# zyj0021200/simpleImageCaptionZoo

Hardware: AMD Instinct MI355X
Metric: captions/sec (SCST step), BUTDDetection COCO14-size vocab (higher is better)
Workload: dtype f32

## Files before the change

include/icz.h:

```cpp
#ifndef ICZ_H_
#define ICZ_H_
#include <stddef.h>
#include <stdint.h>

#ifdef __cplusplus
extern "C" {
#endif

typedef enum {
    ICZ_OK = 0,
    ICZ_ERR_INVALID = -1,
    ICZ_ERR_HIP = -2,
    ICZ_ERR_STATE = -3,
    ICZ_ERR_NOMEM = -4
} icz_status;

const char* icz_last_error(void);
const char* icz_version(void);

typedef struct icz_butd icz_butd_t;

typedef struct {
    int32_t R;
    int32_t D;
// ... 233 lines not shown
int icz_rouge_lcs(const int32_t* hyp_tok, const int32_t* hyp_ptr, const int32_t* ref_tok, const int32_t* ref_ptr,
                  const int32_t* img_ref_ptr, int32_t n_img, int32_t* lcs_out, void* stream);

int icz_gemm_f32(int32_t layout, const float* X, int32_t ldx, const float* W, int32_t ldw, const float* bias,
                 float* C, int32_t ldc, int32_t M, int32_t N, int32_t K, int32_t nsplit, float* workspace,
                 size_t workspace_floats, void* stream);
size_t icz_gemm_workspace_floats(int32_t M, int32_t N);
int icz_gemm_set_big_cfg(int32_t cfg);
int icz_gemm_big_cfg_for(int32_t layout, int32_t M, int32_t N, int32_t K, int32_t nsplit);
int icz_gemm_tn_grouped(const float* dY, int32_t ldy, int32_t M, int32_t K, int32_t ngroups, const float* const* X, const int32_t* ldx,
                        const int32_t* cols, float* const* out, const int32_t* ldo, const int32_t* rows_live, void* stream);
int icz_gemm_tn_split_pick(int32_t M, int32_t N, int32_t K);
int icz_gemm_tn_split(const float* dY, int32_t ldy, int32_t M, const float* X, int32_t ldx, int32_t N, int32_t K, float* out, int32_t ldo,
                      float* workspace, size_t workspace_floats, const int32_t* rows_live, void* stream);
int icz_gemm_route_for(int32_t layout, int32_t M, int32_t N, int32_t nseg, const int32_t* K, int32_t nsplit);
int icz_gemm_tn_grouped_fits(int32_t M, int32_t K, int32_t ngroups, const int32_t* cols);
int icz_prof_begin(void);
int icz_prof_select(int32_t which);
int icz_prof_pair_overhead(void* stream, int32_t n, double* avg_us);
int icz_prof_end(double* avg_us, double* bytes_per_launch, double* flops_per_launch, long long* launches);
int icz_kprof_begin(void);
int icz_kprof_end(int32_t group, double* avg_us, long long* pairs);
int icz_prof_stream_rate(const void* buf, size_t bytes, int32_t reps, void* stream, double* gbs);

#ifdef __cplusplus
}
#endif
#endif
```

simpleimagecaptionzoo_amd/_lib.py:

```python
import ctypes as C
import os

_HERE = os.path.dirname(os.path.abspath(__file__))
LIB_PATH = os.path.join(_HERE, "libicz.so")


class IczError(RuntimeError):
    pass


GRAD_READY_CB = C.CFUNCTYPE(None, C.c_void_p, C.c_int32)


class ButdDims(C.Structure):
    _fields_ = [(n, C.c_int32) for n in ("R", "D", "H", "E", "A", "V", "max_rows", "max_len")]


BUTD_PARAM_FIELDS = (
    "embed_weight",
    "td_w_ih", "td_w_hh", "td_b_ih", "td_b_hh",
    "lm_w_ih", "lm_w_hh", "lm_b_ih", "lm_b_hh",
    "enc_att_v", "enc_att_g", "enc_att_b",
    "dec_att_v", "dec_att_g", "dec_att_b",
    "affine_v", "affine_g", "affine_b",
# ... 176 lines not shown
        "icz_prof_pair_overhead": (C.c_int, [vp, i32, C.POINTER(C.c_double)]),
        "icz_prof_end": (C.c_int, [C.POINTER(C.c_double), C.POINTER(C.c_double), C.POINTER(C.c_double), C.POINTER(C.c_longlong)]),
        "icz_kprof_begin": (C.c_int, []),
        "icz_kprof_end": (C.c_int, [i32, C.POINTER(C.c_double), C.POINTER(C.c_longlong)]),
        "icz_prof_stream_rate": (C.c_int, [vp, C.c_size_t, i32, vp, C.POINTER(C.c_double)]),
        "icz_adam_clamp_multi": (C.c_int, [i32, C.POINTER(vp), C.POINTER(vp), C.POINTER(vp), C.POINTER(vp), C.POINTER(i64), f32, f32, i32, vp]),
        "icz_gemm_f32": (C.c_int, [i32, vp, i32, vp, i32, vp, vp, i32, i32, i32, i32, i32, vp, C.c_size_t, vp]),
        "icz_gemm_workspace_floats": (C.c_size_t, [i32, i32]),
        "icz_gemm_set_big_cfg": (C.c_int, [i32]),
        "icz_gemm_big_cfg_for": (C.c_int, [i32, i32, i32, i32, i32]),
        "icz_gemm_tn_grouped": (C.c_int, [vp, i32, i32, i32, i32, vp, vp, vp, vp, vp, vp, vp]),
        "icz_gemm_tn_split_pick": (C.c_int, [i32, i32, i32]),
        "icz_gemm_tn_split": (C.c_int, [vp, i32, i32, vp, i32, i32, i32, vp, i32, vp, C.c_size_t, vp, vp]),
        "icz_gemm_route_for": (C.c_int, [i32, i32, i32, i32, vp, i32]),
        "icz_gemm_tn_grouped_fits": (C.c_int, [i32, i32, i32, vp]),
    }
    for name, (res, args) in sig.items():
        try:
            fn = getattr(L, name)
        except AttributeError as e:
            raise IczError("libicz.so lacks symbol %s (stale build?)" % name) from e
        fn.restype, fn.argtypes = res, args
    _lib = L
    return L


def check(status):
    if status != 0:
        raise IczError("libicz status %d: %s" % (status, lib().icz_last_error().decode()))

# ... 9 lines not shown
```

simpleimagecaptionzoo_amd/butd.py:

```python
import ctypes as C

import torch

from . import _lib
from ._lib import BUTD_PARAM_KEYS, ButdDims, ButdParams, Rng, check, lib, ptr, stream_ptr
from .handle import GraphDecoderHandle


def make_rng(seed=0, uniforms=None, emb_mask=None, att_mask=None, out_mask=None):
    r = Rng()
    r.seed = int(seed) & 0xFFFFFFFFFFFFFFFF
    keep = []
    for name, t, dt in (("uniforms", uniforms, torch.float32), ("emb_mask", emb_mask, torch.uint8),
                        ("att_mask", att_mask, torch.uint8), ("out_mask", out_mask, torch.uint8)):
        if t is not None:
            if t.dtype != dt or not t.is_cuda or not t.is_contiguous():
                raise _lib.IczError("%s must be a contiguous %s CUDA tensor" % (name, dt))
            setattr(r, name, t.data_ptr())
            keep.append(t)
    r._keep = keep
    return r


class ButdHandle(GraphDecoderHandle):
# ... 82 lines not shown
        N = W.shape[0]
    elif layout == "nn":
        M, K = X.shape
        N = W.shape[1]
    else:
        K, M = X.shape
        N = W.shape[1]
    out = torch.empty(M, N, device=X.device, dtype=torch.float32)
    ws = torch.empty(max(lib().icz_gemm_workspace_floats(M, N), max(nsplit, 1) * M * N), device=X.device,
                     dtype=torch.float32)
    check(lib().icz_gemm_f32(code, ptr(X), X.stride(0), ptr(W), W.stride(0), ptr(bias), ptr(out), N, M, N, K,
                             nsplit, ptr(ws), ws.numel(), stream_ptr()))
    return out


def gemm_set_big_cfg(cfg):
    check(lib().icz_gemm_set_big_cfg(int(cfg)))


def gemm_tn_grouped(dY, Xs, outs=None, rows_live=None):
    K, M = dY.shape
    n = len(Xs)
    if outs is None:
        outs = [torch.empty(M, x.shape[1], device=dY.device, dtype=torch.float32) for x in Xs]
    xp = (C.c_void_p * n)(*[x.data_ptr() for x in Xs])
    op = (C.c_void_p * n)(*[o.data_ptr() for o in outs])
    ldx = (C.c_int32 * n)(*[x.stride(0) for x in Xs])
    cols = (C.c_int32 * n)(*[x.shape[1] for x in Xs])
    ldo = (C.c_int32 * n)(*[o.stride(0) for o in outs])
    check(lib().icz_gemm_tn_grouped(ptr(dY), dY.stride(0), M, K, n, xp, ldx, cols, op, ldo, ptr(rows_live), stream_ptr()))
# ... 34 lines not shown
```

simpleimagecaptionzoo_amd/csrc/butd.hip:

```cpp
#include <vector>

#include "butd_impl.h"

namespace icz {

int Butd::init(const icz_butd_dims& d) {
    dims = d;
    ICZ_REQUIRE(d.R > 0 && d.R <= 64, "butd: R=%d must be in 1..64 (36 boxes / 49 grid cells)", d.R);
    ICZ_REQUIRE(d.D % 4 == 0 && d.H % 4 == 0 && d.E % 4 == 0 && d.A % 4 == 0, "butd: D,H,E,A must be multiples of 4");
    ICZ_REQUIRE(d.V > 3 && d.max_rows > 0 && d.max_len > 0, "butd: bad V/max_rows/max_len");
    const size_t rows = d.max_rows, H = d.H, D = d.D, E = d.E, A = d.A, V = d.V, R = d.R;
    ICZ_TRY(alloc((void**)&w_enc, sizeof(float) * A * D));
    ICZ_TRY(alloc((void**)&w_dec, sizeof(float) * A * H));
    ICZ_TRY(alloc((void**)&w_aff, sizeof(float) * A));
    const size_t Vp = pad_vocab(d.V);
    ICZ_TRY(alloc((void**)&w_pred, sizeof(float) * Vp * H));
    ICZ_TRY(alloc((void**)&n_enc, sizeof(float) * A));
    ICZ_TRY(alloc((void**)&n_dec, sizeof(float) * A));
    ICZ_TRY(alloc((void**)&n_aff, sizeof(float) * 4));
    ICZ_TRY(alloc((void**)&n_pred, sizeof(float) * V));
    ICZ_TRY(alloc((void**)&mean, sizeof(float) * rows * D));
    ICZ_TRY(alloc((void**)&premean, sizeof(float) * rows * 4 * H));
    ICZ_TRY(alloc((void**)&enc_ctx, sizeof(float) * rows * R * A));
    for (int i = 0; i < 2; ++i) {
// ... 13 lines not shown
    ICZ_TRY(alloc((void**)&it, sizeof(int64_t) * rows));
    ICZ_TRY(alloc_scalars(mem));
    size_t nmax = 4 * H;
    if (A > nmax) nmax = A;
    if (V > nmax) nmax = V;
    ws_floats = (size_t)TARGET_WGS * 4096 * 2 + rows * nmax;
    {
        const size_t kmax = 2 * H + (E > D ? E : D), r128 = rows < 128 ? rows : 128;
        const size_t need = (kmax / 256 + 1) * r128 * 4 * H;
        if (need > ws_floats) ws_floats = need;
    }
    ICZ_TRY(alloc((void**)&ws, sizeof(float) * ws_floats));
    ICZ_TRY(mem.synced());
    if (const char* e = getenv("ICZ_EARLY_OUT")) early_out = atoi(e) != 0;
    if (const char* e = getenv("ICZ_MERGE_SMALL")) { const int n = atoi(e); if (n >= 0 && n <= 32) merge_small = n; }
    return ICZ_OK;
}

int Butd::refresh(hipStream_t st) {
    ICZ_REQUIRE(bound, "butd: parameters not bound");
    const int A = dims.A, D = dims.D, H = dims.H, V = dims.V;
    WeightNormTable wt = {};
    int nb = 0;
    auto add = [&](const float* v, const float* g, float* w, float* norm, int rows, int cols) {
        wt.j[wt.count++] = {v, g, w, norm, rows, cols, nb};
        nb += cdiv(rows, 4);
    };
    add(P.enc_att_v, P.enc_att_g, w_enc, n_enc, A, D);
    add(P.dec_att_v, P.dec_att_g, w_dec, n_dec, A, H);
    add(P.affine_v, P.affine_g, w_aff, n_aff, 1, A);
    add(P.predict_v, P.predict_g, w_pred, n_pred, V, H);
    hipLaunchKernelGGL(weight_norm_multi_kernel, dim3(nb), dim3(256), 0, st, wt);
    ICZ_CHECK_HIP(hipGetLastError());
    fresh = true;
    wt_fresh = false;
    return ICZ_OK;
}

bool Butd::wt_possible() const {
    GemmArgs g = {};
    g.nseg = 1;
    g.seg[0] = {w_enc, w_enc, 4 * dims.H, 4 * dims.H, 4 * dims.H, nullptr};
    g.M = 64; g.N = dims.D + dims.H;
    GemmArgs p = g, q = g;
    p.N = q.N = dims.H;
    p.nseg = 2; p.seg[1] = p.seg[0];
    return dims.H % 64 == 0 && dims.D % 64 == 0 && gemm_resident_x3_fits(g) && gemm_resident_x3_pair_fits(p, q);
}

int Butd::refresh_transposes(hipStream_t st) {
    ICZ_REQUIRE(bound && wt_lm_ih, "butd: no transposed weight buffers");
    const int H = dims.H, D = dims.D, E = dims.E;
    TransposeTable tt = {};
    int nb = 0;
    auto add = [&](const float* src, int ld, int cols, float* dst) {
        tt.j[tt.count++] = {src, ld, 4 * H, cols, dst, nb};
        nb += (4 * H / 64) * (cols / 64);
    };
    add(P.lm_w_ih, D + H, D + H, wt_lm_ih);
    add(P.lm_w_hh, H, H, wt_lm_hh);
    add(P.td_w_ih, H + D + E, H, wt_td_ih_h2);
    add(P.td_w_hh, H, H, wt_td_hh);
// ... 231 lines not shown
        b->gc.clear();
    }
    b->P = *p;
    b->bound = true;
    b->fresh = false;
    return ICZ_OK;
}

int icz_butd_set_option(icz_butd_t* h, const char* name, int32_t value) {
    ICZ_REQUIRE(h && name, "icz_butd_set_option: null argument");
    Butd* b = reinterpret_cast<Butd*>(h);
    if (strcmp(name, "graphs") == 0) { b->use_graphs = value != 0; return ICZ_OK; }
    if (strcmp(name, "concurrent") == 0) { b->concurrent = value != 0; return ICZ_OK; }
    if (strcmp(name, "early_out") == 0) { b->early_out = value != 0; return ICZ_OK; }
    if (strcmp(name, "small_nt") == 0) { b->small_nt = value != 0; return ICZ_OK; }
    if (strcmp(name, "group_att") == 0) { b->group_att = value != 0; return ICZ_OK; }
    if (strcmp(name, "merge_small") == 0) {
        ICZ_REQUIRE(value >= 0 && value <= 32, "icz_butd_set_option: merge_small %d outside 0..32", value);
        b->merge_small = value;
        return ICZ_OK;
    }
    set_error("icz_butd_set_option: unknown option '%s'", name);
    return ICZ_ERR_INVALID;
}

int icz_butd_set_mask_sum_global(icz_butd_t* h, const float* mask_sum_global_dev, void* stream) {
    return set_norm_global("icz_butd_set_mask_sum_global", reinterpret_cast<Butd*>(h), mask_sum_global_dev, stream);
}

int icz_butd_set_grad_callback(icz_butd_t* h, icz_grad_ready_cb cb, void* user) {
// ... 40 lines not shown
```

simpleimagecaptionzoo_amd/csrc/butd_impl.h:

```cpp
#pragma once
#include <vector>
#include <stdint.h>

#include "decoder_core.h"

namespace icz {

struct StepIO {
    int rows;
    const float* feats;
    const int32_t* img_of_row;
    int rows_per_img;
    const int64_t* it;
    bool emb_ready;
    const float *h1_in, *c1_in, *h2_in, *c2_in;
    float *h1_out, *c1_out, *h2_out, *c2_out;
    float* emb_out;
    float* gates_td_out;
    float* gates_lm_out;
    float* dec_ctx_out;
    float* alpha_out;
    float* alpha_out2; int alpha2_stride;
    float* ctx_out;
    float* h2drop_out;
// ... 32 lines not shown
    icz_butd_params P;
    bool bound = false, fresh = false;
    DeviceBuffers mem;

    float *w_enc = nullptr, *w_dec = nullptr, *w_aff = nullptr, *w_pred = nullptr;
    float *n_enc = nullptr, *n_dec = nullptr, *n_aff = nullptr, *n_pred = nullptr;
    float *mean = nullptr, *premean = nullptr, *enc_ctx = nullptr;
    float *h1[2], *c1[2], *h2[2], *c2[2];
    float *emb = nullptr, *ctx = nullptr, *scores = nullptr, *alpha = nullptr, *h2drop = nullptr, *logits = nullptr;
    int64_t* it = nullptr;
    float* amax_val = nullptr; int* amax_idx = nullptr;
    float* ws = nullptr;
    size_t ws_floats = 0;
    float *wt_lm_ih = nullptr, *wt_lm_hh = nullptr, *wt_td_ih_h2 = nullptr, *wt_td_hh = nullptr;
    bool wt_fresh = false;
    bool wt_possible() const;
    int refresh_transposes(hipStream_t st);

    int alloc(void** p, size_t bytes) { return mem.alloc(p, bytes); }
    int init(const icz_butd_dims& d);
    int refresh(hipStream_t st);
    int gemm_nt(GemmArgs& g, int* nsplit_out, hipStream_t st);
    int prologue(const float* feats, int n_img, hipStream_t st);
    int step(const StepIO& s, hipStream_t st);
    int zero_state(int rows, int which, hipStream_t st);
    int greedy(const float* feats, int B, int max_len, int64_t* ids_out, float* alphas_out, hipStream_t st);

    GraphCache gc{24};
    bool use_graphs = false;
    bool concurrent = true;
    uintptr_t opt_bits() const {
        return (concurrent ? 1 : 0) + (early_out ? 2 : 0) + 4 * merge_small + (small_nt ? 256 : 0) + (group_att ? 512 : 0);
    }
    int greedy_impl(const float* feats, int B, int max_len, int64_t* ids_out, float* alphas_out, hipStream_t st);
    int sample_impl(const float* feats, int B, int T, int64_t* seq_out, float* logp_out, hipStream_t st);
    int greedy_chain(const float* feats, int B, int max_len, int64_t* ids_out, float* alphas_out, hipStream_t st, bool scst = false);
    int sample_chain(const float* feats, int B, int T, int64_t* seq_out, float* logp_out, hipStream_t st, int row0 = 0, int64_t* ids_out = nullptr);
    int rollouts(const float* feats, int B, int T, const icz_rng* r, int64_t* ids_out, int64_t* seq_out, float* logp_out, hipStream_t st);
    int rollouts_impl(const float* feats, int B, int T, int64_t* ids_out, int64_t* seq_out, float* logp_out, hipStream_t st);
    SideStream side;
    SideStream low;
    icz_grad_ready_cb grad_cb = nullptr; void* grad_cb_user = nullptr;
    int sample_backward_impl(const float* reward, const icz_butd_params& G, float* loss_out, float* mask_sum_out, hipStream_t st,
                             int phases = 0xF, bool fire_cb = true);
    bool bptt_joined = false;
    int merge_small = 8;
    int cur_rows = 0, cur_row0 = 0;
    bool early_out = true;
    bool bptt_early_out = false;
    bool small_nt = true;
    int cur_K = 1, cur_nimg = 0;
    bool group_att = false;

    const float* seam_feats = nullptr;
    int vocab() const override { return dims.V; }
    int row_capacity() const override { return dims.max_rows; }
    bool refreshed() const override { return fresh; }
    bool compact_step() const override { return true; }
    EmbSlot emb_slot() const override { return {P.embed_weight, emb, dims.E, 1}; }
    DeviceBuffers& buffers() override { return mem; }
    int prologue(const float* feats, int n_img, int k, const int32_t* img_of_row, hipStream_t st) override;
    int step(int rows, const int64_t* it, const int32_t* img_of_row, int rows_per_img, int cur, bool slabs, LogitsView* out,
             hipStream_t st) override;
    void gather(const int32_t* src_row, int rows, int fan, hipStream_t st) override;
// ... 27 lines not shown
```

simpleimagecaptionzoo_amd/csrc/butd_kernels.h:

```cpp
#pragma once
#include <stdlib.h>

#include "icz_common.h"
#include "rng.h"

namespace icz {
namespace {

__global__ __launch_bounds__(256) void weight_norm_kernel(const float* __restrict__ v, const float* __restrict__ g,
                                                          float* __restrict__ w, float* __restrict__ norm,
                                                          int rows, int cols) {
    const int lane = threadIdx.x & 63;
    const int row = blockIdx.x * 4 + (threadIdx.x >> 6);
    if (row >= rows) return;
    const float* vr = v + (size_t)row * cols;
    float ss = 0.f;
    for (int c = lane * 4; c < cols; c += 256) {
        f32x4 x = *reinterpret_cast<const f32x4*>(vr + c);
        ss += x[0] * x[0] + x[1] * x[1] + x[2] * x[2] + x[3] * x[3];
    }
    ss = wave_sum(ss);
    const float nrm = sqrtf(ss);
    const float s = g[row] / nrm;
    float* wr = w + (size_t)row * cols;
// ... 1194 lines not shown
    int lda_a;
    const float* dh_b; int ns_b; int lda_b;
    const float* dh_c; int ns_c; int lda_c;
    const float* dhdrop;
    const float* dc_in;
    const float* gates;
    const float* c_prev;
    const float* c_cur;
    float* dgates;
    float* dc_prev;
    int rows, H;
    int rows_a, rows_b, rows_c;
    int dc_in_rows;
    const int* live;
    const int* carry_live;
};
__global__ __launch_bounds__(256) void lstm_bwd_point_kernel(LstmBwdArgs a, DropCfg dc) {
    const int row = blockIdx.y;
    const int j = blockIdx.x * 256 + threadIdx.x;
    if (j >= a.H) return;
    const int H = a.H, G = 4 * H;
    const int lflag = live_flag(a.live), cflag = live_flag(a.carry_live);
    const float* g = a.gates + (size_t)row * G + j;
    const float gi = g[0], gf = g[H], gg = g[2 * H], go = g[3 * H];
    const float cc = a.c_cur[(size_t)row * H + j];
    const float cp = a.c_prev ? a.c_prev[(size_t)row * H + j] : 0.f;
    float dhd = 0.f;
    if (a.dhdrop) dhd = a.dhdrop[(size_t)row * H + j];
    if (flag_dead(lflag)) {
        float* o = a.dgates + (size_t)row * G + j;
        o[0] = 0.f; o[H] = 0.f; o[2 * H] = 0.f; o[3 * H] = 0.f;
        return;
    }
    const bool carry = cflag != 0;
    float dh = 0.f;
    if (a.dh_a && carry && row < a.rows_a) dh += sum_slabs1(a.dh_a, a.ns_a, (size_t)a.rows_a * a.lda_a, (size_t)row * a.lda_a + j);
    if (a.dh_b && row < a.rows_b) dh += sum_slabs1(a.dh_b, a.ns_b, (size_t)a.rows_b * a.lda_b, (size_t)row * a.lda_b + j);
    if (a.dh_c && row < a.rows_c) dh += sum_slabs1(a.dh_c, a.ns_c, (size_t)a.rows_c * a.lda_c, (size_t)row * a.lda_c + j);
    if (a.dhdrop) {
        float d = dhd;
        if (dc.mode) d = dc.keep((uint64_t)row * H + j) ? d * 2.0f : 0.f;
        dh += d;
    }
    const float dcin = (a.dc_in && carry && row < a.dc_in_rows) ? a.dc_in[(size_t)row * H + j] : 0.f;
    const float tc = tanhf(cc);
    const float dcv = dcin + dh * go * (1.f - tc * tc);
    float* o = a.dgates + (size_t)row * G + j;
    o[0] = dcv * gg * gi * (1.f - gi);
    o[H] = dcv * cp * gf * (1.f - gf);
    o[2 * H] = dcv * gi * (1.f - gg * gg);
    o[3 * H] = dh * tc * go * (1.f - go);
// ... 647 lines not shown
```

simpleimagecaptionzoo_amd/csrc/butd_train.hip:

```cpp
#include <math.h>

#include "butd_impl.h"

namespace icz {

static inline int round4(int x) { return pad_vocab(x); }

__global__ void sample_init_kernel(uint8_t* unf, int* nunf, int64_t* tok, int B, int T) {
    const int i = blockIdx.x * blockDim.x + threadIdx.x;
    if (i < B) { unf[i] = 1; tok[i] = 1; }
    if (i < T) nunf[i] = 0;
}

int Butd::ensure_train(int B, int T) {
    if (tb.B >= B && tb.T >= T) return ICZ_OK;
    ICZ_REQUIRE(B <= 2 * dims.max_rows, "butd: batch %d exceeds capacity %d", B, dims.max_rows);
    ICZ_REQUIRE(T <= XE_MAX_T, "butd: %d steps exceed the limit of %d", T, XE_MAX_T);
    if (tb.B > B) B = tb.B;
    if (tb.T > T) T = tb.T;
    if (dims.max_len > T) T = dims.max_len;
    if (!mem.training.empty()) {
        ICZ_TRY(mem.release_training(&gc));
        tb = TrainBuf();
        drop_loss_buffers();
    }
    if (!wt_lm_ih && wt_possible()) {
        const size_t G4 = 4 * (size_t)dims.H;
        ICZ_TRY(alloc((void**)&wt_lm_ih, sizeof(float) * G4 * (dims.D + dims.H)));
        ICZ_TRY(alloc((void**)&wt_lm_hh, sizeof(float) * G4 * dims.H));
        ICZ_TRY(alloc((void**)&wt_td_ih_h2, sizeof(float) * G4 * dims.H));
        ICZ_TRY(alloc((void**)&wt_td_hh, sizeof(float) * G4 * dims.H));
        wt_fresh = false;
    }
    DeviceBuffers::TrainingScope scope(mem);
    const size_t H = dims.H, D = dims.D, E = dims.E, A = dims.A, R = dims.R, V = dims.V;
    const size_t Vp = round4(dims.V);
    const size_t TB = (size_t)T * B;
    ICZ_TRY(alloc((void**)&tb.tok, sizeof(int64_t) * (TB + B)));
    ICZ_TRY(alloc((void**)&tb.emb, sizeof(float) * TB * E));
    ICZ_TRY(alloc((void**)&tb.h1, sizeof(float) * (TB + B) * H));
    ICZ_TRY(alloc((void**)&tb.c1, sizeof(float) * (TB + B) * H));
    ICZ_TRY(alloc((void**)&tb.h2, sizeof(float) * (TB + B) * H));
    ICZ_TRY(alloc((void**)&tb.c2, sizeof(float) * (TB + B) * H));
    ICZ_TRY(alloc((void**)&tb.gtd, sizeof(float) * TB * 4 * H));
    ICZ_TRY(alloc((void**)&tb.glm, sizeof(float) * TB * 4 * H));
    ICZ_TRY(alloc((void**)&tb.dec, sizeof(float) * TB * A));
// ... 440 lines not shown
        }
    }
    ICZ_TRY(side_branch());
    const bool ragged = rows_t[T - 1] < B || roff > 0;
    if (ragged) {
        ICZ_CHECK_HIP(hipMemsetAsync(tb.dGtd, 0, sizeof(float) * (size_t)TB * 4 * H, st));
        ICZ_CHECK_HIP(hipMemsetAsync(tb.dGlm, 0, sizeof(float) * (size_t)TB * 4 * H, st));
        ICZ_CHECK_HIP(hipMemsetAsync(tb.dDec, 0, sizeof(float) * (size_t)TB * A, st));
        ICZ_CHECK_HIP(hipMemsetAsync(tb.dS, 0, sizeof(float) * (size_t)TB * R, st));
    }

    auto loop = [&]() -> int {
    int cur = 0;
    int ns1 = 1, ns2 = 1, ns3 = 1, ns4 = 1;
    int bnext = 0;
    for (int t = T - 1; t >= 0; --t) {
        const int bt = rows_t[t];
        const size_t slot = (size_t)t * Bs + roff;
        const int* const live = (bptt_early_out && early_out && t > 0) ? nunf + (t - 1) : nullptr;
        const int* const carry_live = (bptt_early_out && early_out && t + 1 < T) ? nunf + t : nullptr;
        DropCfg d_out = make_drop(d_seed, cur_train, rng.out_mask, (size_t)B * H, RNG_OUT, t);
        DropCfg d_att = make_drop(d_seed, cur_train, rng.att_mask, (size_t)B * R * A, RNG_ATT, t);
        DropCfg d_off = {0, nullptr, nullptr, 0, 0};
        {
            LstmBwdArgs a = {};
            a.dh_a = bnext ? tb.X[2] : nullptr; a.ns_a = ns3; a.lda_a = H; a.rows_a = bnext;
            a.dhdrop = tb.dH2d + slot * H;
            a.dc_in = bnext ? tb.dc2[cur] : nullptr; a.dc_in_rows = bnext;
            a.gates = tb.glm + slot * 4 * H;
            a.c_prev = tb.c2 + slot * H; a.c_cur = tb.c2 + slot * H + sH;
            a.dgates = tb.dGlm + slot * 4 * H; a.dc_prev = tb.dc2[cur ^ 1];
            a.rows = bt; a.H = H; a.live = live; a.carry_live = carry_live;
            hipLaunchKernelGGL(lstm_bwd_point_kernel, dim3(cdiv(H, 256), bt), dim3(256), 0, st, a, d_out);
        }
        const bool rdg = wt_lm_ih && wt_fresh && bt > 32 && bt <= 64 && gemm_slab_floats(bt, D + H, 4 * H / 256) <= tb.xfloats &&
                         gemm_slab_floats(bt, H, 2 * (4 * H / 256)) <= tb.xfloats;
        const bool tdg = small_nt && wt_lm_ih && wt_fresh && bt <= 32;
        if (rdg) {
            GemmArgs g = {};
            g.nseg = 1;
            g.seg[0] = {tb.dGlm + slot * 4 * H, wt_lm_ih, 4 * H, 4 * H, 4 * H, nullptr};
            g.M = bt; g.N = D + H; g.out = tb.X[0]; g.ldo = D + H; g.live = live;
            g.nsplit = ns1 = gemm_resident_x3_nsplit(g);
            ICZ_REQUIRE(gemm_slab_floats(bt, D + H, ns1) <= tb.xfloats, "butd: slab buffer too small for the dgrad slabs");
            ICZ_TRY(gemm_f32(GEMM_NT, g, st));
        } else if (tdg) {
            GemmArgs g = {};
            g.nseg = 1;
            g.seg[0] = {tb.dGlm + slot * 4 * H, wt_lm_ih, 4 * H, 4 * H, 4 * H, nullptr};
            g.M = bt; g.N = D + H; g.out = tb.X[0]; g.ldo = D + H; g.live = live;
            ICZ_TRY(gemm_auto(GEMM_NT, g, tb.X[0], tb.xfloats, &ns1, st));
        } else {
            GemmArgs g = {};
            g.nseg = 1;
            g.seg[0] = {tb.dGlm + slot * 4 * H, P.lm_w_ih, 4 * H, D + H, 4 * H, nullptr};
            g.M = bt; g.N = D + H; g.out = tb.X[0]; g.ldo = D + H; g.live = live;
            ICZ_TRY(gemm_auto(GEMM_NN, g, tb.X[0], tb.xfloats, &ns1, st));
        }
        {
            const int dparts = cdiv(D, DALPHA_COLS);
            hipLaunchKernelGGL(att_bwd_dalpha_kernel, dim3(bt, dparts), dim3(256), 0, st, tb.X[0], ns1, D + H, bt, feats, R, D, tb.dalpha, live, imgk);
            AttBwdDdecArgs da = {enc_ctx, tb.dec + slot * A, w_aff, tb.alpha + slot * R, tb.dalpha, tb.dDec + slot * A, tb.dS + slot * R, R, A, dparts, live, imgk};
            hipLaunchKernelGGL(att_bwd_ddec_kernel, dim3(bt, cdiv(A, 256)), dim3(256), 0, st, da, d_att);
            GemmArgs g = {};
            g.nseg = 1;
            g.seg[0] = {tb.dDec + slot * A, w_dec, A, H, A, nullptr};
            g.M = bt; g.N = H; g.out = tb.X[1]; g.ldo = H; g.live = live;
            ICZ_TRY(gemm_auto(GEMM_NN, g, tb.X[1], tb.xfloats, &ns2, st));
        }
        {
            LstmBwdArgs a = {};
            a.dh_a = bnext ? tb.X[3] : nullptr; a.ns_a = ns4; a.lda_a = H; a.rows_a = bnext;
            a.dh_b = tb.X[0] + D; a.ns_b = ns1; a.lda_b = D + H; a.rows_b = bt;
            a.dh_c = tb.X[1]; a.ns_c = ns2; a.lda_c = H; a.rows_c = bt;
            a.dc_in = bnext ? tb.dc1[cur] : nullptr; a.dc_in_rows = bnext;
            a.gates = tb.gtd + slot * 4 * H;
            a.c_prev = tb.c1 + slot * H; a.c_cur = tb.c1 + slot * H + sH;
            a.dgates = tb.dGtd + slot * 4 * H; a.dc_prev = tb.dc1[cur ^ 1];
            a.rows = bt; a.H = H; a.live = live; a.carry_live = carry_live;
            hipLaunchKernelGGL(lstm_bwd_point_kernel, dim3(cdiv(H, 256), bt), dim3(256), 0, st, a, d_off);
        }
        if (t > 0 && rdg) {
            GemmArgs g3 = {}, g4 = {};
            g3.nseg = 2;
            g3.seg[0] = {tb.dGlm + slot * 4 * H, wt_lm_hh, 4 * H, 4 * H, 4 * H, nullptr};
            g3.seg[1] = {tb.dGtd + slot * 4 * H, wt_td_ih_h2, 4 * H, 4 * H, 4 * H, nullptr};
            g3.M = bt; g3.N = H; g3.out = tb.X[2]; g3.ldo = H; g3.live = live;
            g4.nseg = 1; g4.live = live;
            g4.seg[0] = {tb.dGtd + slot * 4 * H, wt_td_hh, 4 * H, 4 * H, 4 * H, nullptr};
            g4.M = bt; g4.N = H; g4.out = tb.X[3]; g4.ldo = H;
            ns3 = gemm_resident_x3_nsplit(g3); ns4 = gemm_resident_x3_nsplit(g4);
            ICZ_REQUIRE(gemm_slab_floats(bt, H, ns3) <= tb.xfloats, "butd: slab buffer too small for the dgrad slabs");
            ICZ_TRY(gemm_resident_x3_pair(g3, g4, st));
        } else if (t > 0 && tdg) {
            {
                GemmArgs g = {};
                g.nseg = 2;
// ... 14 lines not shown
                GemmArgs g = {};
                g.nseg = 2;
                g.seg[0] = {tb.dGlm + slot * 4 * H, P.lm_w_hh, 4 * H, H, 4 * H, nullptr};
                g.seg[1] = {tb.dGtd + slot * 4 * H, P.td_w_ih, 4 * H, H + D + E, 4 * H, nullptr};
                g.M = bt; g.N = H; g.out = tb.X[2]; g.ldo = H; g.live = live;
                ICZ_TRY(gemm_auto(GEMM_NN, g, tb.X[2], tb.xfloats, &ns3, st));
            }
            {
                GemmArgs g = {};
                g.nseg = 1;
                g.seg[0] = {tb.dGtd + slot * 4 * H, P.td_w_hh, 4 * H, H, 4 * H, nullptr};
                g.M = bt; g.N = H; g.out = tb.X[3]; g.ldo = H; g.live = live;
                ICZ_TRY(gemm_auto(GEMM_NN, g, tb.X[3], tb.xfloats, &ns4, st));
            }
        }
        bnext = bt;
        cur ^= 1;
    }
    return ICZ_OK;
    };
    const int s_loop = loop();
    if (grad_cb || s_loop != ICZ_OK) {
        ICZ_CHECK_HIP(hipStreamWaitEvent(st, ev_join, 0));
        bptt_joined = true;
    }
    if (s_loop != ICZ_OK) return s_loop;
    }
    if ((phases & 1) && grad_cb && fire_cb) grad_cb(grad_cb_user, 0);
    const int ldtd = H + D + E, ldlm = D + H;
    const bool tail_side = phases == 0xF && !grad_cb && concurrent;
// ... 218 lines not shown
```

simpleimagecaptionzoo_amd/csrc/gemm_f32.h:

```cpp
#pragma once
#include "icz_common.h"

namespace icz {

constexpr int GEMM_MAX_SEG = 4;
constexpr int GEMM_BM = 64, GEMM_BN = 64, GEMM_BK = 64;

enum GemmLayout { GEMM_NT = 0, GEMM_NN = 1, GEMM_TN = 2 };

struct GemmSeg {
    const float* A;
    const float* B;
    int lda, ldb;
    int K;
    const int64_t* gather;
};

struct GemmArgs {
    GemmSeg seg[GEMM_MAX_SEG];
    int nseg;
    int M, N;
    float* out;
    int ldo;
    const float* bias;
    int nsplit;
    int chunks_per_split;
    int accumulate;
    int spread;
    const int* live;
    const int* rows_live;
};

int gemm_f32(GemmLayout layout, const GemmArgs& a, hipStream_t stream);
int gemm_route(GemmLayout layout, const GemmArgs& a);
int gemm_pick_split(const GemmArgs& a, int target_wgs, GemmLayout layout = GEMM_NT);
int gemm_pick_split_balanced(const GemmArgs& a, GemmLayout layout, size_t slab_capacity_floats);
size_t gemm_slab_floats(int M, int N, int nsplit);
int gemm_normalize_split(GemmLayout layout, const GemmArgs& a, int nsplit);
int gemm_fit_split(GemmLayout layout, const GemmArgs& a, int nsplit, size_t capacity_floats);

bool gemm_resident_x3_fits(const GemmArgs& a);
int gemm_resident_x3_stages(const GemmArgs& a);
int gemm_resident_x3_nsplit(const GemmArgs& a);
int gemm_resident_x3(const GemmArgs& a, hipStream_t stream);
bool gemm_resident_x3_pair_fits(const GemmArgs& a, const GemmArgs& b);
int gemm_resident_x3_pair(const GemmArgs& a, const GemmArgs& b, hipStream_t stream);
int gemm_predict(const float* x, int H, const float* w_pred, const float* bias, int rows, int V, int Vp, float* logits, int ldl,
                 float* ws, size_t ws_cap_floats, int* pred_nsplit, hipStream_t st, const int* live = nullptr);

int gemm_big_x3(GemmLayout layout, const GemmArgs& a, int cfg, hipStream_t stream);
int gemm_big_cfg(GemmLayout layout, const GemmArgs& a);
int gemm_big_switch();
void gemm_set_big_cfg(int cfg);
constexpr int GEMM_MAX_COLGROUPS = 4;
struct GemmColGroup { const float* B; int ldb; int cols; float* out; int ldo; };
bool gemm_tn_grouped_fits(int M, int K, const GemmColGroup* groups, int ngroups);
int gemm_tn_grouped(const float* dY, int ldy, int M, int K, const GemmColGroup* groups, int ngroups, const int* rows_live, hipStream_t stream);

// ... 7 lines not shown
```

simpleimagecaptionzoo_amd/csrc/gemm_f32.hip:

```cpp
#include <stdlib.h>

#include <array>
#include <mutex>
#include <set>
#include <vector>

#include "gemm_f32.h"
#include "butd_kernels.h"

namespace icz {

static int total_chunks(const GemmArgs& a, int bk = GEMM_BK) {
    int t = 0;
    for (int s = 0; s < a.nseg; ++s) t += cdiv(a.seg[s].K, bk);
    return t;
}

template <int BK>
struct ChunkCursorT {
    int seg, k0;
    const float* A; const float* B;
    int lda, ldb, K;
    __device__ __forceinline__ void load_seg(const GemmArgs& a) {
        const GemmSeg& g = a.seg[seg];
// ... 1215 lines not shown
    if (g.nsplit > 1) {
        ICZ_REQUIRE(workspace, "icz_gemm_f32: split-K needs a workspace");
        ICZ_REQUIRE(gemm_slab_floats(M, N, g.nsplit) <= workspace_floats, "icz_gemm_f32: workspace of %zu floats too small for %d slabs of %dx%d", workspace_floats, g.nsplit, M, N);
        ICZ_REQUIRE(ldc == N, "icz_gemm_f32: split-K path needs ldc == N");
        g.out = workspace; g.bias = nullptr;
        ICZ_TRY(gemm_f32((GemmLayout)layout, g, st));
        size_t MN = (size_t)M * N;
        ICZ_REQUIRE(MN % 4 == 0, "icz_gemm_f32: M*N must be a multiple of 4 for the split-K reduce");
        hipLaunchKernelGGL(slab_reduce_kernel, dim3(cdiv((int)(MN / 4), 256)), dim3(256), 0, st, workspace, g.nsplit, MN, N, bias, C);
        ICZ_CHECK_HIP(hipGetLastError());
        return ICZ_OK;
    }
    return gemm_f32((GemmLayout)layout, g, st);
}

int icz_gemm_set_big_cfg(int32_t cfg) {
    ICZ_REQUIRE(cfg >= -2 && cfg <= 5, "icz_gemm_set_big_cfg: %d", cfg);
    gemm_set_big_cfg(cfg);
    return ICZ_OK;
}

int icz_gemm_big_cfg_for(int32_t layout, int32_t M, int32_t N, int32_t K, int32_t nsplit) {
    if (layout < 0 || layout > 2 || M <= 0 || N <= 0 || K <= 0) return -1;
    GemmArgs g = {};
    g.nseg = 1;
    g.seg[0].K = K;
    g.M = M; g.N = N; g.nsplit = nsplit > 0 ? nsplit : 1;
    return gemm_big_cfg((GemmLayout)layout, g);
}

// ... 51 lines not shown
```

simpleimagecaptionzoo_amd/csrc/gemm_resident_x3.hip:

```cpp
#include <stdlib.h>

#include <type_traits>

#include "gemm_f32.h"

namespace icz {

template <int I, int N, class F>
__device__ __forceinline__ void sk_static_for(F&& f) {
    if constexpr (I < N) {
        f(std::integral_constant<int, I>{});
        sk_static_for<I + 1, N>(f);
    }
}

typedef __attribute__((ext_vector_type(8))) __bf16 sk_bf16x8;
typedef __attribute__((ext_vector_type(4))) uint32_t sk_u32x4;
typedef __attribute__((ext_vector_type(2))) uint32_t sk_u32x2;

__device__ __forceinline__ uint32_t sk_cvt_pk_bf16(float lo, float hi) {
    uint32_t r;
    asm("v_cvt_pk_bf16_f32 %0, %1, %2" : "=v"(r) : "v"(lo), "v"(hi));
    return r;
}
// ... 491 lines not shown
}

template <int D, bool STAMPS = false>
__global__ __launch_bounds__(256) void gemm_resident_x3_m128_kernel(GemmArgs a) {
    resident_x3_m128_body<D, STAMPS>(a, blockIdx.x);
}
constexpr size_t rs_m128_lds_bytes() { return (size_t)3 * 128 * rs_pb(2) * 2; }

static int rs_total_stages(const GemmArgs& a) {
    int tot = 0;
    for (int s = 0; s < a.nseg; ++s) tot += a.seg[s].K / SK_BK;
    return tot;
}
int gemm_resident_x3_stages(const GemmArgs& a) {
    const int tot = rs_total_stages(a);
    if (gemm_switches().resident_k512 && a.M <= 64 && tot % 8 == 0) return 8;
    return tot % 4 == 0 ? 4 : 0;
}
static bool rs_shape_ok(const GemmArgs& a) {
    if (!gemm_switches().resident_x3 || a.M <= 32 || a.M > (gemm_switches().resident_m128 ? 128 : 64) || a.N % 4 || a.accumulate) return false;
    for (int s = 0; s < a.nseg; ++s)
        if (a.seg[s].K % SK_BK || a.seg[s].gather) return false;
    return rs_total_stages(a) >= 8 && gemm_resident_x3_stages(a) > 0;
}
bool gemm_resident_x3_fits(const GemmArgs& a) { return a.N >= 2048 && rs_shape_ok(a); }
int gemm_resident_x3_nsplit(const GemmArgs& a) { return rs_total_stages(a) / gemm_resident_x3_stages(a); }

template <int NSR, bool STAMPS>
static int rs_launch(const GemmArgs& a, hipStream_t stream) {
    constexpr size_t lds = rs_lds_bytes<4, NSR>();
    static bool attr = false;
    if (!attr) {
        ICZ_CHECK_HIP(hipFuncSetAttribute(reinterpret_cast<const void*>(gemm_resident_x3_kernel<4, NSR, 2, 3, STAMPS>), hipFuncAttributeMaxDynamicSharedMemorySize, (int)lds));
        attr = true;
    }
    hipLaunchKernelGGL((gemm_resident_x3_kernel<4, NSR, 2, 3, STAMPS>), dim3(cdiv(a.N, 256) * a.nsplit), dim3(256), lds, stream, a);
    ICZ_CHECK_HIP(hipGetLastError());
    return ICZ_OK;
}

#ifndef RS_K512_D
#define RS_K512_D 3
#endif
template <bool STAMPS>
static int rs_launch_k512(const GemmArgs& a, hipStream_t stream) {
    constexpr size_t lds = rs_lds_bytes<4, 4>();
    static bool attr = false;
    if (!attr) {
        ICZ_CHECK_HIP(hipFuncSetAttribute(reinterpret_cast<const void*>(gemm_resident_x3_kernel<4, 8, 1, RS_K512_D, STAMPS, 4>), hipFuncAttributeMaxDynamicSharedMemorySize, (int)lds));
        attr = true;
    }
// ... 18 lines not shown
#ifdef ICZ_DEV
static unsigned long long* g_sk_stamps = nullptr;
static int rs_dev_env(const char* name) { const char* e = getenv(name); return e ? atoi(e) : 0; }
#endif

int gemm_resident_x3(const GemmArgs& a_in, hipStream_t stream) {
    GemmArgs a = a_in;
    const int nsr = gemm_resident_x3_stages(a);
    ICZ_REQUIRE(rs_shape_ok(a) && a.nsplit == gemm_resident_x3_nsplit(a) && a.chunks_per_split == nsr,
                "gemm_resident_x3: launch does not match the kernel's fixed decomposition (nsplit %d)", a.nsplit);
    ICZ_REQUIRE(a.nsplit > 1 || a.ldo >= a.N, "gemm_resident_x3: output row stride %d below N = %d", a.ldo, a.N);
#ifdef ICZ_DEV
    if (rs_dev_env("ICZ_DEV_STAMPS")) {
        if (!g_sk_stamps) ICZ_CHECK_HIP(hipMalloc((void**)&g_sk_stamps, sizeof(unsigned long long) * 32 * 4096));
        a.bias = reinterpret_cast<const float*>(g_sk_stamps);
        return a.M > 64 ? rs_launch_m128<true>(a, stream) : (nsr == 8 ? rs_launch_k512<true>(a, stream) : rs_launch<4, true>(a, stream));
    }
#endif
    return a.M > 64 ? rs_launch_m128<false>(a, stream) : (nsr == 8 ? rs_launch_k512<false>(a, stream) : rs_launch<4, false>(a, stream));
}

bool gemm_resident_x3_pair_fits(const GemmArgs& a, const GemmArgs& b) {
    return a.M <= 64 && b.M <= 64 && rs_shape_ok(a) && rs_shape_ok(b) && gemm_resident_x3_stages(a) == gemm_resident_x3_stages(b) && a.N >= 512 && b.N >= 512;
}
int gemm_resident_x3_pair(const GemmArgs& a_in, const GemmArgs& b_in, hipStream_t stream) {
    ICZ_REQUIRE(gemm_resident_x3_pair_fits(a_in, b_in), "gemm_resident_x3_pair: shapes outside the kernel's decomposition");
    GemmPair g;
    g.a = a_in; g.b = b_in;
    const int nsr = gemm_resident_x3_stages(g.a), tilew = nsr == 8 ? 128 : 256;
    for (GemmArgs* p : {&g.a, &g.b}) {
        p->nsplit = gemm_resident_x3_nsplit(*p);
        p->chunks_per_split = nsr;
        p->bias = nullptr;
        ICZ_REQUIRE(p->out && p->nsplit > 1, "gemm_resident_x3_pair: slab output expected");
// ... 44 lines not shown
```

Baseline: 11850.

## Regroup BPTT dgrad GEMMs by concatenating LSTM weight transposes

Stores the transposed LSTM weights contiguously, so the LM input and recurrent dgrads become one wider GEMM (N = D+2H), and the TD input/recurrent dgrads one GEMM of width 2H. It adds a narrow resident-kernel form that uses one tile per workgroup, giving that 2H GEMM more workgroups. The pointwise backward kernel gains a second carried-gradient source so it can read the split slabs. The aim is fewer launches and better occupancy per timestep, at the cost of more slab memory and extra routing logic.

```diff
diff --git a/include/icz.h b/include/icz.h
--- a/include/icz.h
+++ b/include/icz.h
@@ -271,6 +271,8 @@
 int icz_gemm_tn_split(const float* dY, int32_t ldy, int32_t M, const float* X, int32_t ldx, int32_t N, int32_t K, float* out, int32_t ldo,
                       float* workspace, size_t workspace_floats, const int32_t* rows_live, void* stream);
 int icz_gemm_route_for(int32_t layout, int32_t M, int32_t N, int32_t nseg, const int32_t* K, int32_t nsplit);
+int icz_gemm_resident_slabs(const float* X, int32_t ldx, const float* W, int32_t ldw, int32_t M, int32_t N, int32_t K, int32_t form,
+                            float* slabs, size_t slab_floats, int32_t* nsplit_out, void* stream);
 int icz_gemm_tn_grouped_fits(int32_t M, int32_t K, int32_t ngroups, const int32_t* cols);
 int icz_prof_begin(void);
 int icz_prof_select(int32_t which);
diff --git a/simpleimagecaptionzoo_amd/_lib.py b/simpleimagecaptionzoo_amd/_lib.py
--- a/simpleimagecaptionzoo_amd/_lib.py
+++ b/simpleimagecaptionzoo_amd/_lib.py
@@ -214,6 +214,7 @@
         "icz_gemm_tn_split": (C.c_int, [vp, i32, i32, vp, i32, i32, i32, vp, i32, vp, C.c_size_t, vp, vp]),
         "icz_gemm_route_for": (C.c_int, [i32, i32, i32, i32, vp, i32]),
         "icz_gemm_tn_grouped_fits": (C.c_int, [i32, i32, i32, vp]),
+        "icz_gemm_resident_slabs": (C.c_int, [vp, i32, vp, i32, i32, i32, i32, i32, vp, C.c_size_t, C.POINTER(i32), vp]),
     }
     for name, (res, args) in sig.items():
         try:
diff --git a/simpleimagecaptionzoo_amd/butd.py b/simpleimagecaptionzoo_amd/butd.py
--- a/simpleimagecaptionzoo_amd/butd.py
+++ b/simpleimagecaptionzoo_amd/butd.py
@@ -120,6 +120,16 @@
     return out
 
 
+def gemm_resident_slabs(X, W, form=0, max_slabs=64):
+    M, K = X.shape
+    N = W.shape[0]
+    ws = torch.empty(max_slabs * M * N, device=X.device, dtype=torch.float32)
+    ns = C.c_int32(0)
+    check(lib().icz_gemm_resident_slabs(ptr(X), X.stride(0), ptr(W), W.stride(0), M, N, K, int(form), ptr(ws), ws.numel(), C.byref(ns),
+                                        stream_ptr()))
+    return ws[:ns.value * M * N].view(ns.value, M, N)
+
+
 def gemm_set_big_cfg(cfg):
     check(lib().icz_gemm_set_big_cfg(int(cfg)))
 
diff --git a/simpleimagecaptionzoo_amd/csrc/butd.hip b/simpleimagecaptionzoo_amd/csrc/butd.hip
--- a/simpleimagecaptionzoo_amd/csrc/butd.hip
+++ b/simpleimagecaptionzoo_amd/csrc/butd.hip
@@ -51,6 +51,7 @@
     ICZ_TRY(mem.synced());
     if (const char* e = getenv("ICZ_EARLY_OUT")) early_out = atoi(e) != 0;
     if (const char* e = getenv("ICZ_MERGE_SMALL")) { const int n = atoi(e); if (n >= 0 && n <= 32) merge_small = n; }
+    if (const char* e = getenv("ICZ_BPTT_REGROUP")) { const int n = atoi(e); if (n >= 0 && n <= 2) bptt_regroup = n; }
     return ICZ_OK;
 }
 
@@ -79,10 +80,20 @@
     g.nseg = 1;
     g.seg[0] = {w_enc, w_enc, 4 * dims.H, 4 * dims.H, 4 * dims.H, nullptr};
     g.M = 64; g.N = dims.D + dims.H;
-    GemmArgs p = g, q = g;
-    p.N = q.N = dims.H;
-    p.nseg = 2; p.seg[1] = p.seg[0];
-    return dims.H % 64 == 0 && dims.D % 64 == 0 && gemm_resident_x3_fits(g) && gemm_resident_x3_pair_fits(p, q);
+    GemmArgs g2 = g, n = g;
+    g2.N = dims.D + 2 * dims.H;
+    n.N = 2 * dims.H; n.form = GEMM_FORM_NARROW;
+    return dims.H % 64 == 0 && dims.D % 64 == 0 && gemm_resident_x3_fits(g) && gemm_resident_x3_fits(g2) && gemm_resident_x3_takes(n);
+}
+bool Butd::wt_pair_possible() const {
+    GemmArgs p = {};
+    p.nseg = 2;
+    p.seg[0] = {w_enc, w_enc, 4 * dims.H, 4 * dims.H, 4 * dims.H, nullptr};
+    p.seg[1] = p.seg[0];
+    p.M = 64; p.N = dims.H;
+    GemmArgs q = p;
+    q.nseg = 1;
+    return gemm_resident_x3_pair_fits(p, q);
 }
 
 int Butd::refresh_transposes(hipStream_t st) {
@@ -344,6 +355,11 @@
     if (strcmp(name, "concurrent") == 0) { b->concurrent = value != 0; return ICZ_OK; }
     if (strcmp(name, "early_out") == 0) { b->early_out = value != 0; return ICZ_OK; }
     if (strcmp(name, "small_nt") == 0) { b->small_nt = value != 0; return ICZ_OK; }
+    if (strcmp(name, "bptt_regroup") == 0) {
+        ICZ_REQUIRE(value >= 0 && value <= 2, "icz_butd_set_option: bptt_regroup %d outside 0..2", value);
+        b->bptt_regroup = value;
+        return ICZ_OK;
+    }
     if (strcmp(name, "group_att") == 0) { b->group_att = value != 0; return ICZ_OK; }
     if (strcmp(name, "merge_small") == 0) {
         ICZ_REQUIRE(value >= 0 && value <= 32, "icz_butd_set_option: merge_small %d outside 0..32", value);
diff --git a/simpleimagecaptionzoo_amd/csrc/butd_impl.h b/simpleimagecaptionzoo_amd/csrc/butd_impl.h
--- a/simpleimagecaptionzoo_amd/csrc/butd_impl.h
+++ b/simpleimagecaptionzoo_amd/csrc/butd_impl.h
@@ -70,7 +70,9 @@
     size_t ws_floats = 0;
     float *wt_lm_ih = nullptr, *wt_lm_hh = nullptr, *wt_td_ih_h2 = nullptr, *wt_td_hh = nullptr;
     bool wt_fresh = false;
+    bool wt_pair = false;
     bool wt_possible() const;
+    bool wt_pair_possible() const;
     int refresh_transposes(hipStream_t st);
 
     int alloc(void** p, size_t bytes) { return mem.alloc(p, bytes); }
@@ -86,7 +88,7 @@
     bool use_graphs = false;
     bool concurrent = true;
     uintptr_t opt_bits() const {
-        return (concurrent ? 1 : 0) + (early_out ? 2 : 0) + 4 * merge_small + (small_nt ? 256 : 0) + (group_att ? 512 : 0);
+        return (concurrent ? 1 : 0) + (early_out ? 2 : 0) + 4 * merge_small + (small_nt ? 256 : 0) + (group_att ? 512 : 0) + 1024 * bptt_regroup;
     }
     int greedy_impl(const float* feats, int B, int max_len, int64_t* ids_out, float* alphas_out, hipStream_t st);
     int sample_impl(const float* feats, int B, int T, int64_t* seq_out, float* logp_out, hipStream_t st);
@@ -104,6 +106,7 @@
     int cur_rows = 0, cur_row0 = 0;
     bool early_out = true;
     bool bptt_early_out = false;
+    int bptt_regroup = 1;
     bool small_nt = true;
     int cur_K = 1, cur_nimg = 0;
     bool group_att = false;
diff --git a/simpleimagecaptionzoo_amd/csrc/butd_kernels.h b/simpleimagecaptionzoo_amd/csrc/butd_kernels.h
--- a/simpleimagecaptionzoo_amd/csrc/butd_kernels.h
+++ b/simpleimagecaptionzoo_amd/csrc/butd_kernels.h
@@ -1232,6 +1232,8 @@
     int dc_in_rows;
     const int* live;
     const int* carry_live;
+    const float* dh_a2; int ns_a2;
+    int lda_a2;
 };
 __global__ __launch_bounds__(256) void lstm_bwd_point_kernel(LstmBwdArgs a, DropCfg dc) {
     const int row = blockIdx.y;
@@ -1253,6 +1255,7 @@
     const bool carry = cflag != 0;
     float dh = 0.f;
     if (a.dh_a && carry && row < a.rows_a) dh += sum_slabs1(a.dh_a, a.ns_a, (size_t)a.rows_a * a.lda_a, (size_t)row * a.lda_a + j);
+    if (a.dh_a2 && carry && row < a.rows_a) dh += sum_slabs1(a.dh_a2, a.ns_a2, (size_t)a.rows_a * a.lda_a2, (size_t)row * a.lda_a2 + j);
     if (a.dh_b && row < a.rows_b) dh += sum_slabs1(a.dh_b, a.ns_b, (size_t)a.rows_b * a.lda_b, (size_t)row * a.lda_b + j);
     if (a.dh_c && row < a.rows_c) dh += sum_slabs1(a.dh_c, a.ns_c, (size_t)a.rows_c * a.lda_c, (size_t)row * a.lda_c + j);
     if (a.dhdrop) {
diff --git a/simpleimagecaptionzoo_amd/csrc/butd_train.hip b/simpleimagecaptionzoo_amd/csrc/butd_train.hip
--- a/simpleimagecaptionzoo_amd/csrc/butd_train.hip
+++ b/simpleimagecaptionzoo_amd/csrc/butd_train.hip
@@ -26,10 +26,11 @@
     }
     if (!wt_lm_ih && wt_possible()) {
         const size_t G4 = 4 * (size_t)dims.H;
-        ICZ_TRY(alloc((void**)&wt_lm_ih, sizeof(float) * G4 * (dims.D + dims.H)));
-        ICZ_TRY(alloc((void**)&wt_lm_hh, sizeof(float) * G4 * dims.H));
-        ICZ_TRY(alloc((void**)&wt_td_ih_h2, sizeof(float) * G4 * dims.H));
-        ICZ_TRY(alloc((void**)&wt_td_hh, sizeof(float) * G4 * dims.H));
+        ICZ_TRY(alloc((void**)&wt_lm_ih, sizeof(float) * G4 * (dims.D + 2 * dims.H)));
+        wt_lm_hh = wt_lm_ih + G4 * (dims.D + dims.H);
+        ICZ_TRY(alloc((void**)&wt_td_ih_h2, sizeof(float) * G4 * 2 * dims.H));
+        wt_td_hh = wt_td_ih_h2 + G4 * dims.H;
+        wt_pair = wt_pair_possible();
         wt_fresh = false;
     }
     DeviceBuffers::TrainingScope scope(mem);
@@ -500,6 +501,9 @@
     int cur = 0;
     int ns1 = 1, ns2 = 1, ns3 = 1, ns4 = 1;
     int bnext = 0;
+    struct Carry { const float* p; int ns, ld; };
+    Carry lm_c = {nullptr, 1, H}, lm_c2 = {nullptr, 1, H}, td_c = {nullptr, 1, H};
+    const bool wt_ok = wt_lm_ih && wt_fresh && (bptt_regroup || wt_pair);
     for (int t = T - 1; t >= 0; --t) {
         const int bt = rows_t[t];
         const size_t slot = (size_t)t * Bs + roff;
@@ -510,7 +514,8 @@
         DropCfg d_off = {0, nullptr, nullptr, 0, 0};
         {
             LstmBwdArgs a = {};
-            a.dh_a = bnext ? tb.X[2] : nullptr; a.ns_a = ns3; a.lda_a = H; a.rows_a = bnext;
+            a.dh_a = bnext ? lm_c.p : nullptr; a.ns_a = lm_c.ns; a.lda_a = lm_c.ld; a.rows_a = bnext;
+            a.dh_a2 = bnext ? lm_c2.p : nullptr; a.ns_a2 = lm_c2.ns; a.lda_a2 = lm_c2.ld;
             a.dhdrop = tb.dH2d + slot * H;
             a.dc_in = bnext ? tb.dc2[cur] : nullptr; a.dc_in_rows = bnext;
             a.gates = tb.glm + slot * 4 * H;
@@ -519,16 +524,26 @@
             a.rows = bt; a.H = H; a.live = live; a.carry_live = carry_live;
             hipLaunchKernelGGL(lstm_bwd_point_kernel, dim3(cdiv(H, 256), bt), dim3(256), 0, st, a, d_out);
         }
-        const bool rdg = wt_lm_ih && wt_fresh && bt > 32 && bt <= 64 && gemm_slab_floats(bt, D + H, 4 * H / 256) <= tb.xfloats &&
-                         gemm_slab_floats(bt, H, 2 * (4 * H / 256)) <= tb.xfloats;
-        const bool tdg = small_nt && wt_lm_ih && wt_fresh && bt <= 32;
+        GemmArgs g1 = {}, g2 = {};
+        g1.nseg = 1;
+        g1.seg[0] = {tb.dGlm + slot * 4 * H, wt_lm_ih, 4 * H, 4 * H, 4 * H, nullptr};
+        g1.M = bt; g1.N = (bptt_regroup && t > 0) ? D + 2 * H : D + H; g1.out = tb.X[0]; g1.ldo = g1.N; g1.live = live;
+        g2.nseg = 1;
+        g2.seg[0] = {tb.dGtd + slot * 4 * H, wt_td_ih_h2, 4 * H, 4 * H, 4 * H, nullptr};
+        g2.M = bt; g2.N = 2 * H; g2.out = tb.X[2]; g2.ldo = 2 * H; g2.live = live;
+        g2.form = bptt_regroup == 1 ? GEMM_FORM_NARROW : GEMM_FORM_AUTO;
+        const bool rows_rdg = wt_ok && bt > 32 && bt <= 64;
+        const bool rdg = rows_rdg && (bptt_regroup
+            ? gemm_resident_x3_fits(g1) && gemm_resident_x3_takes(g2) && gemm_slab_floats(bt, g1.N, gemm_resident_x3_nsplit(g1)) <= tb.xfloats &&
+              gemm_slab_floats(bt, 2 * H, gemm_resident_x3_nsplit(g2)) <= tb.xfloats
+            : gemm_slab_floats(bt, D + H, 4 * H / 256) <= tb.xfloats && gemm_slab_floats(bt, H, 2 * (4 * H / 256)) <= tb.xfloats);
+        const bool regrouped = rdg && bptt_regroup;
+        const int ld1 = regrouped ? g1.N : D + H;
+        const bool tdg = small_nt && wt_ok && bt <= 32;
         if (rdg) {
-            GemmArgs g = {};
-            g.nseg = 1;
-            g.seg[0] = {tb.dGlm + slot * 4 * H, wt_lm_ih, 4 * H, 4 * H, 4 * H, nullptr};
-            g.M = bt; g.N = D + H; g.out = tb.X[0]; g.ldo = D + H; g.live = live;
+            GemmArgs g = g1;
             g.nsplit = ns1 = gemm_resident_x3_nsplit(g);
-            ICZ_REQUIRE(gemm_slab_floats(bt, D + H, ns1) <= tb.xfloats, "butd: slab buffer too small for the dgrad slabs");
+            ICZ_REQUIRE(gemm_slab_floats(bt, g.N, ns1) <= tb.xfloats, "butd: slab buffer too small for the dgrad slabs");
             ICZ_TRY(gemm_f32(GEMM_NT, g, st));
         } else if (tdg) {
             GemmArgs g = {};
@@ -545,7 +560,7 @@
         }
         {
             const int dparts = cdiv(D, DALPHA_COLS);
-            hipLaunchKernelGGL(att_bwd_dalpha_kernel, dim3(bt, dparts), dim3(256), 0, st, tb.X[0], ns1, D + H, bt, feats, R, D, tb.dalpha, live, imgk);
+            hipLaunchKernelGGL(att_bwd_dalpha_kernel, dim3(bt, dparts), dim3(256), 0, st, tb.X[0], ns1, ld1, bt, feats, R, D, tb.dalpha, live, imgk);
             AttBwdDdecArgs da = {enc_ctx, tb.dec + slot * A, w_aff, tb.alpha + slot * R, tb.dalpha, tb.dDec + slot * A, tb.dS + slot * R, R, A, dparts, live, imgk};
             hipLaunchKernelGGL(att_bwd_ddec_kernel, dim3(bt, cdiv(A, 256)), dim3(256), 0, st, da, d_att);
             GemmArgs g = {};
@@ -556,8 +571,8 @@
         }
         {
             LstmBwdArgs a = {};
-            a.dh_a = bnext ? tb.X[3] : nullptr; a.ns_a = ns4; a.lda_a = H; a.rows_a = bnext;
-            a.dh_b = tb.X[0] + D; a.ns_b = ns1; a.lda_b = D + H; a.rows_b = bt;
+            a.dh_a = bnext ? td_c.p : nullptr; a.ns_a = td_c.ns; a.lda_a = td_c.ld; a.rows_a = bnext;
+            a.dh_b = tb.X[0] + D; a.ns_b = ns1; a.lda_b = ld1; a.rows_b = bt;
             a.dh_c = tb.X[1]; a.ns_c = ns2; a.lda_c = H; a.rows_c = bt;
             a.dc_in = bnext ? tb.dc1[cur] : nullptr; a.dc_in_rows = bnext;
             a.gates = tb.gtd + slot * 4 * H;
@@ -566,7 +581,13 @@
             a.rows = bt; a.H = H; a.live = live; a.carry_live = carry_live;
             hipLaunchKernelGGL(lstm_bwd_point_kernel, dim3(cdiv(H, 256), bt), dim3(256), 0, st, a, d_off);
         }
-        if (t > 0 && rdg) {
+        if (t > 0 && regrouped) {
+            GemmArgs g = g2;
+            g.nsplit = ns3 = gemm_resident_x3_nsplit(g);
+            g.chunks_per_split = gemm_resident_x3_stages(g);
+            ICZ_REQUIRE(gemm_slab_floats(bt, 2 * H, ns3) <= tb.xfloats, "butd: slab buffer too small for the dgrad slabs");
+            ICZ_TRY(gemm_resident_x3(g, st));
+        } else if (t > 0 && rdg) {
             GemmArgs g3 = {}, g4 = {};
             g3.nseg = 2;
             g3.seg[0] = {tb.dGlm + slot * 4 * H, wt_lm_hh, 4 * H, 4 * H, 4 * H, nullptr};
@@ -611,6 +632,15 @@
                 ICZ_TRY(gemm_auto(GEMM_NN, g, tb.X[3], tb.xfloats, &ns4, st));
             }
         }
+        if (regrouped) {
+            lm_c = {tb.X[0] + D + H, ns1, ld1};
+            lm_c2 = {tb.X[2], ns3, 2 * H};
+            td_c = {tb.X[2] + H, ns3, 2 * H};
+        } else {
+            lm_c = {tb.X[2], ns3, H};
+            lm_c2 = {nullptr, 1, H};
+            td_c = {tb.X[3], ns4, H};
+        }
         bnext = bt;
         cur ^= 1;
     }
diff --git a/simpleimagecaptionzoo_amd/csrc/gemm_f32.h b/simpleimagecaptionzoo_amd/csrc/gemm_f32.h
--- a/simpleimagecaptionzoo_amd/csrc/gemm_f32.h
+++ b/simpleimagecaptionzoo_amd/csrc/gemm_f32.h
@@ -29,7 +29,9 @@
     int spread;
     const int* live;
     const int* rows_live;
+    int form;
 };
+enum GemmForm { GEMM_FORM_AUTO = 0, GEMM_FORM_NARROW = 1 };
 
 int gemm_f32(GemmLayout layout, const GemmArgs& a, hipStream_t stream);
 int gemm_route(GemmLayout layout, const GemmArgs& a);
@@ -42,6 +44,7 @@
 bool gemm_resident_x3_fits(const GemmArgs& a);
 int gemm_resident_x3_stages(const GemmArgs& a);
 int gemm_resident_x3_nsplit(const GemmArgs& a);
+bool gemm_resident_x3_takes(const GemmArgs& a);
 int gemm_resident_x3(const GemmArgs& a, hipStream_t stream);
 bool gemm_resident_x3_pair_fits(const GemmArgs& a, const GemmArgs& b);
 int gemm_resident_x3_pair(const GemmArgs& a, const GemmArgs& b, hipStream_t stream);
diff --git a/simpleimagecaptionzoo_amd/csrc/gemm_f32.hip b/simpleimagecaptionzoo_amd/csrc/gemm_f32.hip
--- a/simpleimagecaptionzoo_amd/csrc/gemm_f32.hip
+++ b/simpleimagecaptionzoo_amd/csrc/gemm_f32.hip
@@ -1253,6 +1253,23 @@
     return gemm_f32((GemmLayout)layout, g, st);
 }
 
+int icz_gemm_resident_slabs(const float* X, int32_t ldx, const float* W, int32_t ldw, int32_t M, int32_t N, int32_t K, int32_t form,
+                            float* slabs, size_t slab_floats, int32_t* nsplit_out, void* stream) {
+    ICZ_REQUIRE(X && W && slabs && nsplit_out && M > 0 && N > 0 && K > 0 && ldx >= K && ldw >= K, "icz_gemm_resident_slabs: bad arguments");
+    ICZ_REQUIRE(form == GEMM_FORM_AUTO || form == GEMM_FORM_NARROW, "icz_gemm_resident_slabs: form %d (0 = automatic, 1 = narrow)", form);
+    GemmArgs g = {};
+    g.nseg = 1;
+    g.seg[0] = {X, W, ldx, ldw, K, nullptr};
+    g.M = M; g.N = N; g.out = slabs; g.ldo = N; g.form = form;
+    ICZ_REQUIRE(M <= 64 && gemm_resident_x3_takes(g), "icz_gemm_resident_slabs: %d x %d x %d is not taken by the resident kernel in form %d", M, N, K, form);
+    g.nsplit = gemm_resident_x3_nsplit(g);
+    g.chunks_per_split = gemm_resident_x3_stages(g);
+    const size_t need = g.nsplit > 1 ? gemm_slab_floats(M, N, g.nsplit) : (size_t)M * N;
+    ICZ_REQUIRE(need <= slab_floats, "icz_gemm_resident_slabs: %zu floats needed for %d slabs of %d x %d, %zu given", need, g.nsplit, M, N, slab_floats);
+    *nsplit_out = g.nsplit;
+    return gemm_resident_x3(g, (hipStream_t)stream);
+}
+
 int icz_gemm_set_big_cfg(int32_t cfg) {
     ICZ_REQUIRE(cfg >= -2 && cfg <= 5, "icz_gemm_set_big_cfg: %d", cfg);
     gemm_set_big_cfg(cfg);
diff --git a/simpleimagecaptionzoo_amd/csrc/gemm_resident_x3.hip b/simpleimagecaptionzoo_amd/csrc/gemm_resident_x3.hip
--- a/simpleimagecaptionzoo_amd/csrc/gemm_resident_x3.hip
+++ b/simpleimagecaptionzoo_amd/csrc/gemm_resident_x3.hip
@@ -529,27 +529,30 @@
 }
 int gemm_resident_x3_stages(const GemmArgs& a) {
     const int tot = rs_total_stages(a);
+    if (a.form == GEMM_FORM_NARROW) return (a.M <= 64 && tot % 4 == 0) ? 4 : 0;
     if (gemm_switches().resident_k512 && a.M <= 64 && tot % 8 == 0) return 8;
     return tot % 4 == 0 ? 4 : 0;
 }
 static bool rs_shape_ok(const GemmArgs& a) {
     if (!gemm_switches().resident_x3 || a.M <= 32 || a.M > (gemm_switches().resident_m128 ? 128 : 64) || a.N % 4 || a.accumulate) return false;
+    if (a.form != GEMM_FORM_AUTO && a.form != GEMM_FORM_NARROW) return false;
     for (int s = 0; s < a.nseg; ++s)
         if (a.seg[s].K % SK_BK || a.seg[s].gather) return false;
     return rs_total_stages(a) >= 8 && gemm_resident_x3_stages(a) > 0;
 }
 bool gemm_resident_x3_fits(const GemmArgs& a) { return a.N >= 2048 && rs_shape_ok(a); }
+bool gemm_resident_x3_takes(const GemmArgs& a) { return rs_shape_ok(a); }
 int gemm_resident_x3_nsplit(const GemmArgs& a) { return rs_total_stages(a) / gemm_resident_x3_stages(a); }
 
-template <int NSR, bool STAMPS>
+template <int NSR, int TPW, bool STAMPS>
 static int rs_launch(const GemmArgs& a, hipStream_t stream) {
     constexpr size_t lds = rs_lds_bytes<4, NSR>();
     static bool attr = false;
     if (!attr) {
-        ICZ_CHECK_HIP(hipFuncSetAttribute(reinterpret_cast<const void*>(gemm_resident_x3_kernel<4, NSR, 2, 3, STAMPS>), hipFuncAttributeMaxDynamicSharedMemorySize, (int)lds));
+        ICZ_CHECK_HIP(hipFuncSetAttribute(reinterpret_cast<const void*>(gemm_resident_x3_kernel<4, NSR, TPW, 3, STAMPS>), hipFuncAttributeMaxDynamicSharedMemorySize, (int)lds));
         attr = true;
     }
-    hipLaunchKernelGGL((gemm_resident_x3_kernel<4, NSR, 2, 3, STAMPS>), dim3(cdiv(a.N, 256) * a.nsplit), dim3(256), lds, stream, a);
+    hipLaunchKernelGGL((gemm_resident_x3_kernel<4, NSR, TPW, 3, STAMPS>), dim3(cdiv(a.N, 128 * TPW) * a.nsplit), dim3(256), lds, stream, a);
     ICZ_CHECK_HIP(hipGetLastError());
     return ICZ_OK;
 }
@@ -598,10 +601,14 @@
     if (rs_dev_env("ICZ_DEV_STAMPS")) {
         if (!g_sk_stamps) ICZ_CHECK_HIP(hipMalloc((void**)&g_sk_stamps, sizeof(unsigned long long) * 32 * 4096));
         a.bias = reinterpret_cast<const float*>(g_sk_stamps);
-        return a.M > 64 ? rs_launch_m128<true>(a, stream) : (nsr == 8 ? rs_launch_k512<true>(a, stream) : rs_launch<4, true>(a, stream));
+        if (a.M > 64) return rs_launch_m128<true>(a, stream);
+        if (nsr == 8) return rs_launch_k512<true>(a, stream);
+        return a.form == GEMM_FORM_NARROW ? rs_launch<4, 1, true>(a, stream) : rs_launch<4, 2, true>(a, stream);
     }
 #endif
-    return a.M > 64 ? rs_launch_m128<false>(a, stream) : (nsr == 8 ? rs_launch_k512<false>(a, stream) : rs_launch<4, false>(a, stream));
+    if (a.M > 64) return rs_launch_m128<false>(a, stream);
+    if (nsr == 8) return rs_launch_k512<false>(a, stream);
+    return a.form == GEMM_FORM_NARROW ? rs_launch<4, 1, false>(a, stream) : rs_launch<4, 2, false>(a, stream);
 }
 
 bool gemm_resident_x3_pair_fits(const GemmArgs& a, const GemmArgs& b) {
```

New measurement: 11960, median of 6. No clear change (+1.0%).
